# vigorbird/ORB_SLAM2_comment

Measured on AMD Instinct MI355X. Metric: frames/sec ORB extract+match, KITTI 1241×376 @1000 feat; HBM GB/s vs peak, higher is better.
Workload: dtype u8; 1 GPU; configs[1]+[2]+[3]: a global batch of 512 synthetic 1241x376 u8 frames per step, 512 per GPU, resident in HBM as (last, cur) pairs; per step ORB extract (nFeatures=1000, 8-level pyramid) of every frame + device-resident SearchByProjection(CurrentFrame, LastFrame, th=15, mono; projection prologue included) for every pair; monocular handles: mvImagePyramid[0] on demand (orbhip_extractor_set_lazy_lev; handles_per_gpu=3, stage_gates=0, global_batch=512, nfeatures=1000, levels=8, parallelism=pair-sharded x1

## Files before the change

orb_slam2_comment_amd/csrc/orbhip_extractor.hip:

```cpp
#include "orbhip_internal.h"
#include "rbrief_pattern.h"

#include <cfloat>
#include <climits>
#include <cmath>
#include <ctime>
#include <mutex>
#include <new>
#include <vector>

namespace orbhip {

static thread_local char g_err[512] = "";
void set_error(const char *fmt, ...)
{
    va_list ap;
    va_start(ap, fmt);
    vsnprintf(g_err, sizeof(g_err), fmt, ap);
    va_end(ap);
}

__device__ __forceinline__ int wave_reduce_add(int v) { return wave_sum(v); }

template <int T>
// ... 1081 lines not shown
                int spos = incl - surv_cnt;
                for (int i = i_lo; i < i_hi; ++i) {
                    const int r = S.rnk[i];
                    const bool split = r != 0xffff && r <= J;
                    if (!split) {
                        const int ni = Gc + spos++;
                        S.nmap[i] = ni;
                        S.x0[nxt][ni] = S.x0[cur][i]; S.x1[nxt][ni] = S.x1[cur][i];
                        S.y0[nxt][ni] = S.y0[cur][i]; S.y1[nxt][ni] = S.y1[cur][i];
                        S.cnt[nxt][ni] = S.cnt[cur][i];
                    } else {
                        S.nmap[i] = 0x40000000;
                        const int px0 = S.x0[cur][i], px1 = S.x1[cur][i], py0 = S.y0[cur][i], py1 = S.y1[cur][i];
                        const int mx = px0 + ((px1 - px0 + 1) >> 1), my = py0 + ((py1 - py0 + 1) >> 1);
                        int g = r > 0 ? S.cincl[r - 1] : 0;
#pragma unroll
                        for (int q = 0; q < 4; ++q) {
                            const int c = CC[4 * i + q];
                            if (c > 0) {
                                const int ni = Gc - 1 - g;
                                S.x0[nxt][ni] = (short)((q & 1) ? mx : px0);
                                S.x1[nxt][ni] = (short)((q & 1) ? px1 : mx);
                                S.y0[nxt][ni] = (short)((q & 2) ? my : py0);
                                S.y1[nxt][ni] = (short)((q & 2) ? py1 : my);
                                S.cnt[nxt][ni] = c;
                                CC[4 * i + q] = ni;
                                nToExpand += (c > 1);
                                ++g;
                            }
                        }
                    }
                }
            }
            nToExpand = wave_sum(nToExpand);
            const int n_new = Gc + (n - (m > 0 ? J + 1 : 0));
            int fin = 0, ph = phase;
            if (n_new >= N || n_new == prevSize) fin = 1;
            else if (phase == 1 && n_new + nToExpand * 3 > N) ph = 2;
            if (lane == 0) { S.vars[0] = n_new; S.vars[1] = fin; S.vars[2] = ph; }
            int *CN = S.ccnt[cb ^ 1];
            for (int i = lane; i < n_new * 4; i += 64) CN[i] = 0;
        }
        __syncthreads();
        OCT_STAMP(6);
        ++npass;
        if constexpr (REG) {
            oct_sweep<MAXN, T, false>(S, rkey, rlab, K, tid, cur, nxt, CC, S.ccnt[cb ^ 1], false, S.vars[1] == 0);
        } else {
            for (int k0 = 0; k0 < K; k0 += T * kOctU) {
                int nd[kOctU], mp[kOctU];
                uint32_t kv[kOctU];
#pragma unroll
                for (int u = 0; u < kOctU; ++u) {
                    const int k = k0 + u * T + tid;
                    nd[u] = k < K ? (int)knode(k) : 0;
                    kv[u] = k < K ? keys(k) : 0u;
                }
#pragma unroll
                for (int u = 0; u < kOctU; ++u) mp[u] = S.nmap[nd[u]];
                int bx0[kOctU], bx1[kOctU], by0[kOctU], by1[kOctU];
#pragma unroll
                for (int u = 0; u < kOctU; ++u) {
                    bx0[u] = S.x0[cur][nd[u]]; bx1[u] = S.x1[cur][nd[u]];
                    by0[u] = S.y0[cur][nd[u]]; by1[u] = S.y1[cur][nd[u]];
                }
#pragma unroll
                for (int u = 0; u < kOctU; ++u) {
                    const int k = k0 + u * T + tid;
                    if (k >= K) continue;
                    if (mp[u] & 0x40000000) {
                        const int x = kv[u] & 0xfff, y = (kv[u] >> 12) & 0xfff;
                        const int mx = bx0[u] + ((bx1[u] - bx0[u] + 1) >> 1), my = by0[u] + ((by1[u] - by0[u] + 1) >> 1);
                        knode(k) = (unsigned short)CC[4 * nd[u] + (x < mx ? 0 : 1) + (y < my ? 0 : 2)];
                    } else {
                        knode(k) = (unsigned short)mp[u];
                    }
                }
            }
        }
        OCT_STAMP(7);
        n = S.vars[0];
        finish = S.vars[1] != 0;
        phase = S.vars[2];
        cur = nxt;
        cb ^= 1;
    }
    __syncthreads();

    unsigned int *best = reinterpret_cast<unsigned int *>(S.ccnt[0]);
    for (int i = tid; i < n; i += T) best[i] = 0;
    __syncthreads();
    uint32_t *out = sel_kp + (size_t)b * G.kp_cap_total + L.kp_base;
    const int nout = min(n, L.kp_cap);
    if constexpr (REG) {
#pragma unroll
        for (int g = 0; g < kOctR / kOctU; ++g) {
            if (g * kOctU * T < K) {
#pragma unroll
                for (int u = 0; u < kOctU; ++u) {
                    const int k = (g * kOctU + u) * T + tid;
                    if (k < K) atomicMax(&best[oct_nd(rlab, g * kOctU + u)], ((rkey[g * kOctU + u] >> 24) << 24) | (0xffffffu - (uint32_t)k));
                }
            }
        }
        __syncthreads();
#pragma unroll
        for (int g = 0; g < kOctR / kOctU; ++g) {
            if (g * kOctU * T < K) {
                unsigned int bv[kOctU];
#pragma unroll
                for (int u = 0; u < kOctU; ++u) bv[u] = best[oct_nd(rlab, g * kOctU + u)];
#pragma unroll
                for (int u = 0; u < kOctU; ++u) {
                    const int k = (g * kOctU + u) * T + tid, nd = oct_nd(rlab, g * kOctU + u);
                    if (k < K && nd < nout && bv[u] == (((rkey[g * kOctU + u] >> 24) << 24) | (0xffffffu - (uint32_t)k)))
                        out[nd] = rkey[g * kOctU + u];
                }
            }
        }
    } else {
        for (int k0 = 0; k0 < K; k0 += T * kOctU) {
            int nd[kOctU];
            uint32_t kv[kOctU];
#pragma unroll
            for (int u = 0; u < kOctU; ++u) {
                const int k = k0 + u * T + tid;
                nd[u] = k < K ? (int)knode(k) : 0;
                kv[u] = k < K ? keys(k) : 0u;
            }
#pragma unroll
            for (int u = 0; u < kOctU; ++u) {
                const int k = k0 + u * T + tid;
                if (k < K) atomicMax(&best[nd[u]], ((kv[u] >> 24) << 24) | (0xffffffu - (uint32_t)k));
            }
        }
        __syncthreads();
        for (int i = tid; i < nout; i += T) out[i] = keys(0xffffffu - (best[i] & 0xffffffu));
    }
    if (tid == 0) {
        sel_cnt[b * ORBHIP_MAX_LEVELS + level] = nout;
        if (n > L.kp_cap) atomicExch(&frame_status[b], ORBHIP_E_CAPACITY);
    }
    OCT_STAMP(8);
#ifdef ORBHIP_DEVTOOLS
    if constexpr (STAMPS) {
        if (tid == 0 && level == 0) {
#pragma unroll
            for (int i = 0; i < 9; ++i) atomicAdd(&g_oct_stamps[i], tacc[i]);
            atomicAdd(&g_oct_stamps[9], (unsigned long long)npass);
            atomicAdd(&g_oct_stamps[10], 1ull);
            atomicAdd(&g_oct_stamps[11], (unsigned long long)K);
        }
    }
#endif
#undef OCT_STAMP
#undef keys
#undef knode
}

template <int MAXN, int T, bool STAMPS = false>
__global__ __launch_bounds__(T) __attribute__((amdgpu_waves_per_eu(MAXN == 512 && T == 512 ? 8 : 1))) void k_octree(PyrGeom G, const int *__restrict__ cell_cnt,
                                                const uint32_t *__restrict__ cell_kp,
                                                uint32_t *__restrict__ keys_ws,
                                                unsigned short *__restrict__ node_ws,
                                                uint32_t *__restrict__ sel_kp,
                                                int *__restrict__ sel_cnt, int *__restrict__ frame_status,
                                                const int reg_cap)
{
    __shared__ OctShared<MAXN> S;
    unsigned long long t0 = 0;
    if constexpr (STAMPS) t0 = stamp_now();
    int level, b;
    xcd_remap(level, b);
    const int tid = threadIdx.x;
    const LevelGeom L = G.lv[level];
    uint32_t *gkeys = keys_ws + (size_t)b * G.cand_cap_total + L.cand_base;
    unsigned short *gnode = node_ws + (size_t)b * G.cand_cap_total + L.cand_base;
    const int *ccnt_in = cell_cnt + (size_t)b * G.ncells_total + L.cell_base;
    const uint32_t *ckp_in = cell_kp + ((size_t)b * G.ncells_total + L.cell_base) * G.slot_cap;
    int tot;
    int K = 0;
    for (int c0 = 0; c0 < L.ncells; c0 += T) {
        int c = c0 + tid;
        int n = c < L.ncells ? ccnt_in[c] : 0;
        int base = block_excl_scan<T>(n, S.scan, &tot);
        if (c < L.ncells) S.ccnt[0][c] = K + base;
        K += tot;
    }
    K = __builtin_amdgcn_readfirstlane(K);
    if (K <= reg_cap)
        octree_body<MAXN, T, true, STAMPS>(S, G, L, level, b, K, ccnt_in, ckp_in, gkeys, gnode, sel_kp, sel_cnt, frame_status, t0);
    else
        octree_body<MAXN, T, false, STAMPS>(S, G, L, level, b, K, ccnt_in, ckp_in, gkeys, gnode, sel_kp, sel_cnt, frame_status, t0);
}

constexpr int kBIn = kBlurTH + 6;
constexpr int kBInW = 18;

__device__ __forceinline__ uint32_t mad24u(uint32_t a, uint32_t b, uint32_t c)
{
    uint32_t r;
    asm("v_mad_u32_u24 %0, %1, %2, %3" : "=v"(r) : "v"(a), "v"(b), "v"(c));
    return r;
}
__device__ __forceinline__ uint32_t sat_pk_u8(uint32_t v)
{
    uint32_t r;
    asm("v_sat_pk_u8_i16 %0, %1" : "=v"(r) : "v"(v));
    return r;
}

__global__ __launch_bounds__(256) void k_blur(const uint8_t *__restrict__ pyr, uint8_t *__restrict__ blur,
                                              PyrGeom G, const TileDesc *__restrict__ tiles, BlurW W)
{
    __shared__ uint32_t sin[kBIn * kBInW];
    __shared__ uint4 srow[(kBIn / 2) * (kBlurTW / 4)];
    int tile, fr;
    xcd_remap(tile, fr);
    const TileDesc t = tiles[tile];
    const LevelGeom L = G.lv[t.level];
    const size_t fo = (size_t)fr * G.frame_bytes + L.plane_off + (size_t)kEdge * L.pitch + kPadL;
    const uint8_t *roi = pyr + fo;
    uint8_t *out = blur + fo;
    const int x0 = t.tx * kBlurTW, y0 = t.ty * kBlurTH;
    const int rows = min(kBlurTH, L.h - y0);
    const int nin = rows + 6, npair = (nin + 1) >> 1;
    const int tid = threadIdx.x;
    const int gxmax = (L.w + 12) & ~3;
    {
        constexpr int U = (kBIn * kBInW + 255) / 256;
        uint32_t v[U];
#pragma unroll
        for (int u = 0; u < U; ++u) {
            const int i = min(u * 256 + tid, nin * kBInW - 1);
            const int r = (i * 3641) >> 16, c = i - r * kBInW;
            const int gy = min(y0 - 3 + r, L.h + kEdge - 1), gx = min(x0 - 4 + 4 * c, gxmax);
            v[u] = *reinterpret_cast<const uint32_t *>(roi + (ptrdiff_t)(__mul24(gy, L.pitch) + gx));
        }
#pragma unroll
        for (int u = 0; u < U; ++u) {
            const int i = u * 256 + tid;
            if (i < nin * kBInW) sin[i] = v[u];
        }
    }
    const uint32_t B0 = W.w[0], B1 = W.w[1], B2 = W.w[2], B3 = W.w[3], B4 = W.w[4], B5 = W.w[5], B6 = W.w[6];
    const uint32_t k0a = (B0 << 8) | (B1 << 16) | (B2 << 24), k0b = B3 | (B4 << 8) | (B5 << 16) | (B6 << 24);
    const uint32_t k1a = (B0 << 16) | (B1 << 24), k1b = B2 | (B3 << 8) | (B4 << 16) | (B5 << 24), k1c = B6;
    const uint32_t k2a = B0 << 24, k2b = B1 | (B2 << 8) | (B3 << 16) | (B4 << 24), k2c = B5 | (B6 << 8);
    const uint32_t k3b = B0 | (B1 << 8) | (B2 << 16) | (B3 << 24), k3c = B4 | (B5 << 8) | (B6 << 16);
    __syncthreads();
    for (int it = tid; it < npair * 16; it += 256) {
        const int pr = it >> 4, g = it & 15;
        uint32_t s[2][4];
#pragma unroll
        for (int h = 0; h < 2; ++h) {
            const uint32_t *p = &sin[madi24(min(2 * pr + h, nin - 1), kBInW, g)];
            const uint32_t d0 = p[0], d1 = p[1], d2 = p[2];
            s[h][0] = __builtin_amdgcn_udot4(d0, k0a, __builtin_amdgcn_udot4(d1, k0b, 0, false), false);
            s[h][1] = __builtin_amdgcn_udot4(d0, k1a, __builtin_amdgcn_udot4(d1, k1b, __builtin_amdgcn_udot4(d2, k1c, 0, false), false), false);
            s[h][2] = __builtin_amdgcn_udot4(d0, k2a, __builtin_amdgcn_udot4(d1, k2b, __builtin_amdgcn_udot4(d2, k2c, 0, false), false), false);
            s[h][3] = __builtin_amdgcn_udot4(d1, k3b, __builtin_amdgcn_udot4(d2, k3c, 0, false), false);
        }
        srow[it] = make_uint4(__builtin_amdgcn_perm(s[1][0], s[0][0], 0x05040100u), __builtin_amdgcn_perm(s[1][1], s[0][1], 0x05040100u),
                              __builtin_amdgcn_perm(s[1][2], s[0][2], 0x05040100u), __builtin_amdgcn_perm(s[1][3], s[0][3], 0x05040100u));
    }
    __syncthreads();
    const uint32_t w01 = (uint32_t)W.w[0] | ((uint32_t)W.w[1] << 16), w23 = (uint32_t)W.w[2] | ((uint32_t)W.w[3] << 16),
                   w45 = (uint32_t)W.w[4] | ((uint32_t)W.w[5] << 16), w12 = (uint32_t)W.w[1] | ((uint32_t)W.w[2] << 16),
                   w34 = (uint32_t)W.w[3] | ((uint32_t)W.w[4] << 16), w56 = (uint32_t)W.w[5] | ((uint32_t)W.w[6] << 16),
                   w6l = (uint32_t)W.w[6], w0h = (uint32_t)W.w[0] << 16;
    const int nprow = (rows + 1) >> 1;
    for (int it = tid; it < nprow * 16; it += 256) {
        const int p = it >> 4, g = it & 15;
        if (x0 + 4 * g >= L.w) continue;
        const uint4 P0 = srow[p * 16 + g], P1 = srow[(p + 1) * 16 + g], P2 = srow[(p + 2) * 16 + g], P3 = srow[(p + 3) * 16 + g];
        const uint32_t a0[4] = {P0.x, P0.y, P0.z, P0.w}, a1[4] = {P1.x, P1.y, P1.z, P1.w},
                       a2[4] = {P2.x, P2.y, P2.z, P2.w}, a3[4] = {P3.x, P3.y, P3.z, P3.w};
        uint32_t acce[4], acco[4];
#pragma unroll
        for (int j = 0; j < 4; ++j) {
            acce[j] = udot2(a0[j], w01, udot2(a1[j], w23, udot2(a2[j], w45, udot2(a3[j], w6l, 32768u))));
            acco[j] = udot2(a1[j], w12, udot2(a2[j], w34, udot2(a3[j], w56, udot2(a0[j], w0h, 32768u))));
        }
        const uint32_t rese = sat_pk_u8(__builtin_amdgcn_perm(acce[1], acce[0], 0x07060302u)) |
                              (sat_pk_u8(__builtin_amdgcn_perm(acce[3], acce[2], 0x07060302u)) << 16);
        const uint32_t reso = sat_pk_u8(__builtin_amdgcn_perm(acco[1], acco[0], 0x07060302u)) |
                              (sat_pk_u8(__builtin_amdgcn_perm(acco[3], acco[2], 0x07060302u)) << 16);
        uint8_t *o = out + (uint32_t)(__mul24(y0 + 2 * p, L.pitch) + x0 + 4 * g);
        *reinterpret_cast<uint32_t *>(o) = rese;
        if (2 * p + 1 < rows) *reinterpret_cast<uint32_t *>(o + L.pitch) = reso;
    }
}

constexpr int kWinRows = 43, kWinDw = 11;
constexpr int kWinRpi = 5;
constexpr int kWinLoads = 9;
constexpr int kWinWords = kWinRows * kWinDw + 7;
constexpr int kHPairs = 22, kHGroups = 10;

#ifndef ORBHIP_DESC_WAVES
#define ORBHIP_DESC_WAVES 7
#endif
constexpr int kDescWaveSlotsPerCu = 4 * ORBHIP_DESC_WAVES, kDescMinRounds = 6;
static int desc_per_wave(int kp_cap_total, int batch, int num_cus)
{
    const double slots = (double)num_cus * kDescWaveSlotsPerCu;
    for (int p = 4; p > 2; --p)
        if ((double)kp_cap_total * batch / p >= kDescMinRounds * slots) return p;
    return 2;
}

__global__ __launch_bounds__(256) __attribute__((amdgpu_waves_per_eu(ORBHIP_DESC_WAVES, ORBHIP_DESC_WAVES))) void k_describe_fused(const uint8_t *__restrict__ pyr, PyrGeom G,
                                                        const uint32_t *__restrict__ sel_kp,
                                                        const int *__restrict__ sel_cnt,
                                                        const int *__restrict__ desc_tab,
                                                        const float4 *__restrict__ patternf,
                                                        orbhip_keypoint *__restrict__ out_kp,
                                                        uint8_t *__restrict__ out_desc, int cap,
                                                        int *__restrict__ out_n, int *__restrict__ status, int per_wave, BlurW W,
                                                        const uint32_t *__restrict__ hitem_tab,
                                                        const uint8_t *__restrict__ images, int img_stride, size_t img_frame_stride)
{
    __shared__ uint32_t swin[4][kWinWords];
    __shared__ uint4 shsum[4][kHPairs * kHGroups];
    const int lane = threadIdx.x & 63;
    const int wv = __builtin_amdgcn_readfirstlane(threadIdx.x >> 6);
    int bx, b;
    xcd_remap(bx, b);
    int cw[4], uw[4], vw[4];
#pragma unroll
    for (int k = 0; k < 4; ++k) { cw[k] = desc_tab[k * 64 + lane]; uw[k] = desc_tab[256 + k * 64 + lane]; vw[k] = desc_tab[512 + k * 64 + lane]; }
    float4 pat[4];
#pragma unroll
    for (int j = 0; j < 4; ++j) pat[j] = patternf[j * 64 + lane];
    const int *cnts = sel_cnt + b * ORBHIP_MAX_LEVELS;
    int total = 0;
    for (int l = 0; l < G.nlevels; ++l) total += cnts[l];
    if (bx == 0 && wv == 0 && lane == 0) {
        out_n[b] = min(total, cap);
        if (total > cap && status) atomicExch(&status[b], ORBHIP_E_CAPACITY);
    }
    const uint32_t B0 = W.w[0], B1 = W.w[1], B2 = W.w[2], B3 = W.w[3], B4 = W.w[4], B5 = W.w[5], B6 = W.w[6];
    const uint32_t h0a = B0 | (B1 << 8) | (B2 << 16) | (B3 << 24), h0b = B4 | (B5 << 8) | (B6 << 16);
    const uint32_t h1a = (B0 << 8) | (B1 << 16) | (B2 << 24), h1b = B3 | (B4 << 8) | (B5 << 16) | (B6 << 24);
    const uint32_t h2a = (B0 << 16) | (B1 << 24), h2b = B2 | (B3 << 8) | (B4 << 16) | (B5 << 24), h2c = B6;
    const uint32_t h3a = B0 << 24, h3b = B1 | (B2 << 8) | (B3 << 16) | (B4 << 24), h3c = B5 | (B6 << 8);
    const uint32_t w01 = B0 | (B1 << 16), w23 = B2 | (B3 << 16), w45 = B4 | (B5 << 16), w12 = B1 | (B2 << 16),
                   w34 = B3 | (B4 << 16), w56 = B5 | (B6 << 16), w6l = B6, w0h = B0 << 16;
    const int srow = (lane * 373) >> 12, scol = lane - srow * kWinDw;
    const uint32_t hitems = hitem_tab[lane];
    uint32_t *win = swin[wv];
    uint4 *hs = shsum[wv];
  int level = 0, before = 0, mine = 0, kp_base = 0, kp_end = -1, pitch = 0;
  for (int kk = 0; kk < per_wave; ++kk) {
    const int slot = (bx * 4 + wv) * per_wave + kk;
    if (slot >= G.kp_cap_total) break;
    if (slot >= kp_end) {
        level = 0;
        for (int l = 1; l < G.nlevels; ++l) if (slot >= G.lv[l].kp_base) level = l;
        before = 0; mine = 0;
        for (int l = 0; l < G.nlevels; ++l) {
            const int c = cnts[l];
            if (l < level) before += c;
            if (l == level) mine = c;
        }
        kp_base = G.lv[level].kp_base; kp_end = kp_base + G.lv[level].kp_cap; pitch = G.lv[level].pitch;
    }
    const int i = slot - kp_base;
    if (i >= mine) continue;
    const int oidx = before + i;
    if (oidx >= cap) continue;

    const uint32_t kv = sel_kp[(size_t)b * G.kp_cap_total + slot];
    const int kx = (int)(kv & 0xfff) + 16, ky = (int)((kv >> 12) & 0xfff) + 16;
    const int resp = (int)(kv >> 24);
    uint32_t wvv[kWinLoads];
    const bool from_img = images != nullptr && level == 0;
    const bool inside = kx >= 21 && kx + 22 < G.lv[0].w && ky >= 21 && ky + 21 < G.lv[0].h;
    if (from_img && !inside) {
        const uint8_t *ib = images + (size_t)b * img_frame_stride;
        uint32_t cx[4];
#pragma unroll
        for (int k = 0; k < 4; ++k) cx[k] = (uint32_t)reflect101(kx - 21 + 4 * scol + k, G.lv[0].w);
#pragma unroll
        for (int u = 0; u < kWinLoads; ++u) {
            wvv[u] = 0u;
            if (lane < kWinRpi * kWinDw && (u < kWinLoads - 1 || srow < kWinRows - (kWinLoads - 1) * kWinRpi)) {
                const uint8_t *rp = ib + (size_t)((uint32_t)reflect101(ky - 21 + srow + u * kWinRpi, G.lv[0].h) * (uint32_t)img_stride);
                wvv[u] = (uint32_t)rp[cx[0]] | ((uint32_t)rp[cx[1]] << 8) | ((uint32_t)rp[cx[2]] << 16) | ((uint32_t)rp[cx[3]] << 24);
            }
        }
    } else {
        const int wpitch = from_img ? img_stride : pitch;
        const uint8_t *wb = from_img
            ? images + (size_t)b * img_frame_stride + (size_t)(ky - 21) * img_stride + (kx - 21)
            : pyr + (size_t)b * G.frame_bytes + G.lv[level].plane_off + (size_t)kEdge * pitch + kPadL + (size_t)(ky - 21) * pitch + (kx - 21);
        const uint32_t voff = (uint32_t)(__mul24(srow, wpitch) + 4 * scol);
#pragma unroll
        for (int u = 0; u < kWinLoads; ++u) {
            wvv[u] = 0u;
            if (lane < kWinRpi * kWinDw && (u < kWinLoads - 1 || srow < kWinRows - (kWinLoads - 1) * kWinRpi))
                __builtin_memcpy(&wvv[u], wb + (uint32_t)(u * kWinRpi * wpitch) + voff, 4);
        }
    }
    __builtin_amdgcn_wave_barrier();
    if (lane < kWinRpi * kWinDw) {
        uint32_t *dd = win + (srow * kWinDw + scol);
#pragma unroll
        for (int u = 0; u < kWinLoads; ++u)
            if (u < kWinLoads - 1 || srow < kWinRows - (kWinLoads - 1) * kWinRpi) dd[u * kWinRpi * kWinDw] = wvv[u];
    }
    __builtin_amdgcn_wave_barrier();
    int m10 = 0, m01 = 0;
#pragma unroll
    for (int k = 0; k < 4; ++k) {
        const int d = (int)(win[cw[k]] ^ 0x80808080u);
        m10 = __builtin_amdgcn_sdot4(d, uw[k], m10, false);
        m01 = __builtin_amdgcn_sdot4(d, vw[k], m01, false);
    }
#pragma unroll 1
    for (int q = 0; q < 3; ++q) {
        const int it = (int)((hitems >> (8 * q)) & 0xffu);
        const int pr = (it * 205) >> 11, g = it - pr * kHGroups;
        uint32_t s[2][4];
#pragma unroll
        for (int h = 0; h < 2; ++h) {
            const uint32_t *p = &win[madi24(min(2 * pr + h, kWinRows - 1), kWinDw, g)];
            const uint32_t d0 = p[0], d1 = p[1], d2 = p[2];
            s[h][0] = __builtin_amdgcn_udot4(d0, h0a, __builtin_amdgcn_udot4(d1, h0b, 0, false), false);
            s[h][1] = __builtin_amdgcn_udot4(d0, h1a, __builtin_amdgcn_udot4(d1, h1b, 0, false), false);
            s[h][2] = __builtin_amdgcn_udot4(d0, h2a, __builtin_amdgcn_udot4(d1, h2b, __builtin_amdgcn_udot4(d2, h2c, 0, false), false), false);
            s[h][3] = __builtin_amdgcn_udot4(d0, h3a, __builtin_amdgcn_udot4(d1, h3b, __builtin_amdgcn_udot4(d2, h3c, 0, false), false), false);
        }
        hs[it] = make_uint4(__builtin_amdgcn_perm(s[1][0], s[0][0], 0x05040100u), __builtin_amdgcn_perm(s[1][1], s[0][1], 0x05040100u),
                            __builtin_amdgcn_perm(s[1][2], s[0][2], 0x05040100u), __builtin_amdgcn_perm(s[1][3], s[0][3], 0x05040100u));
    }
    m10 = wave_reduce_add(m10);
    m01 = wave_reduce_add(m01);
    const float angle = fast_atan2_deg((float)m01, (float)m10);
    const float factorPI = (float)(3.14159265358979323846 / 180.f);
    float a, bsn;
    det_sincos(__fmul_rn(angle, factorPI), &a, &bsn);
    __builtin_amdgcn_wave_barrier();
    const uint32_t *hd = reinterpret_cast<const uint32_t *>(hs);
    auto round18 = [](float t) -> int {
        return (int)(__float_as_uint(__fadd_rn(t, 12582912.0f)) - (0x4B400000u - 18u));
    };
    uint32_t vw0, vw1, vw2, vw3, vx0, vx1, vx2, vx3;
    asm("v_mov_b32 %0, %1" : "=v"(vw0) : "s"(w01)); asm("v_mov_b32 %0, %1" : "=v"(vx0) : "s"(w01 ^ w0h));
    asm("v_mov_b32 %0, %1" : "=v"(vw1) : "s"(w23)); asm("v_mov_b32 %0, %1" : "=v"(vx1) : "s"(w23 ^ w12));
    asm("v_mov_b32 %0, %1" : "=v"(vw2) : "s"(w45)); asm("v_mov_b32 %0, %1" : "=v"(vx2) : "s"(w45 ^ w34));
    asm("v_mov_b32 %0, %1" : "=v"(vw3) : "s"(w6l)); asm("v_mov_b32 %0, %1" : "=v"(vx3) : "s"(w6l ^ w56));
    auto blurred = [&](int R, int C) -> int {
        const uint32_t *p = hd + madi24(R >> 1, kHGroups * 4, C);
        const uint32_t d0 = p[0], d1 = p[kHGroups * 4], d2 = p[2 * kHGroups * 4], d3 = p[3 * kHGroups * 4];
        const uint32_t om = 0u - (uint32_t)(R & 1);
        const uint32_t acc = udot2(d0, vw0 ^ (om & vx0), udot2(d1, vw1 ^ (om & vx1), udot2(d2, vw2 ^ (om & vx2),
                                   udot2(d3, vw3 ^ (om & vx3), 32768u))));
        return min((int)(acc >> 16), 255);
    };
    unsigned long long bits[4];
    int t0v[4], t1v[4];
#pragma unroll
    for (int j = 0; j < 4; ++j) {
        const float px0 = pat[j].x, py0 = pat[j].y, px1 = pat[j].z, py1 = pat[j].w;
        const int r0 = round18(__fadd_rn(__fmul_rn(px0, bsn), __fmul_rn(py0, a)));
        const int c0 = round18(__fsub_rn(__fmul_rn(px0, a), __fmul_rn(py0, bsn)));
        const int r1 = round18(__fadd_rn(__fmul_rn(px1, bsn), __fmul_rn(py1, a)));
        const int c1 = round18(__fsub_rn(__fmul_rn(px1, a), __fmul_rn(py1, bsn)));
        t0v[j] = blurred(r0, c0);
        t1v[j] = blurred(r1, c1);
    }
#pragma unroll
    for (int j = 0; j < 4; ++j) bits[j] = __ballot(t0v[j] < t1v[j]);
    if (lane < 4) {
        unsigned long long v = lane == 0 ? bits[0] : lane == 1 ? bits[1] : lane == 2 ? bits[2] : bits[3];
        reinterpret_cast<unsigned long long *>(out_desc + ((size_t)b * cap + oidx) * 32)[lane] = v;
    }
    if (lane == 0) {
        orbhip_keypoint kp;
        float fx = (float)kx, fy = (float)ky;
        const float scale = G.lv[level].scale;
        if (level != 0) { fx = __fmul_rn(fx, scale); fy = __fmul_rn(fy, scale); }
        kp.x = fx; kp.y = fy; kp.size = (float)G.lv[level].patch; kp.angle = angle; kp.response = (float)resp;
        kp.octave = level; kp.class_id = -1;
        out_kp[(size_t)b * cap + oidx] = kp;
    }
  }
}

__global__ void k_zero_status(int *status, int n)
{
    int i = blockIdx.x * blockDim.x + threadIdx.x;
    if (i < n) status[i] = 0;
}

}

using namespace orbhip;

#ifdef ORBHIP_DEVTOOLS
#define ORBHIP_STAGE_MASK(e) ((e)->stage_mask)
#else
#define ORBHIP_STAGE_MASK(e) 31
#endif

static int cv_round(double v) { return (int)lrint(v); }

static void drop_graph(orbhip_extractor *e)
{
    if (e->graph_exec) (void)hipGraphExecDestroy(e->graph_exec);
    e->graph_exec = nullptr; e->graph_batch = 0; e->graph_cap = 0;
}
static void free_geometry(orbhip_extractor *e)
{
    drop_graph(e);
    (void)hipFree(e->d_cells); (void)hipFree(e->d_cells2); (void)hipFree(e->d_tiles); (void)hipFree(e->d_pyrtab);
    e->d_cells = nullptr; e->d_cells2 = nullptr; e->d_tiles = nullptr; e->d_pyrtab = nullptr;
    e->bound = false;
}
static void free_batch(orbhip_extractor *e)
{
    drop_graph(e);
    (void)hipFree(e->d_pyr); (void)hipFree(e->d_blur); (void)hipFree(e->d_cell_cnt); (void)hipFree(e->d_cell_kp);
    (void)hipFree(e->d_keys); (void)hipFree(e->d_knode); (void)hipFree(e->d_sel); (void)hipFree(e->d_sel_cnt); (void)hipFree(e->d_status);
    e->d_pyr = e->d_blur = nullptr; e->d_cell_cnt = nullptr; e->d_cell_kp = nullptr; e->d_keys = nullptr;
    e->d_knode = nullptr; e->d_sel = nullptr; e->d_sel_cnt = nullptr; e->d_status = nullptr;
    (void)hipFree(e->d_gray); e->d_gray = nullptr; e->gray_cap = 0;
    e->batch_cap = 0;
    e->blur_valid = false;
}

static void host_resize_coef(int d, double scale, int slen, bool clamp_both, int &s0, int &s1, int &c0, int &c1)
{
#pragma clang fp contract(off)
    const double fd = ((double)d + 0.5) * scale;
    float f = (float)(fd - 0.5);
    int s = (int)floorf(f);
    f = f - (float)s;
    if (clamp_both) {
        s0 = s < 0 ? 0 : (s < slen ? s : slen - 1);
        s1 = s + 1 < 0 ? 0 : (s + 1 < slen ? s + 1 : slen - 1);
    } else {
        if (s < 0) { f = 0.f; s = 0; }
        if (s >= slen - 1) { f = 0.f; s = slen - 1; }
        s0 = s; s1 = s + 1;
    }
    const float g = 1.f - f;
    c0 = (int)lrintf(g * 2048.f);
    c1 = (int)lrintf(f * 2048.f);
}
static int host_reflect101(int p, int len)
{
    if (p < 0) p = -p;
    if (p >= len) p = 2 * (len - 1) - p;
    return p;
}
static void pyr_chunks(PyrLevelTab &T, int rows_per_unit)
{
    T.nchunks = (T.words + 63) / 64;
    T.chunk_w = (T.words + T.nchunks - 1) / T.nchunks;
    T.rcp_chunks = T.nchunks > 1 ? (uint32_t)(((1ull << 32) + (unsigned)T.nchunks - 1) / (unsigned)T.nchunks) : 0u;
    T.units = ((T.prows + rows_per_unit - 1) / rows_per_unit) * T.nchunks;
}

static int build_pyr_tables(orbhip_extractor *e)
{
    const PyrGeom &G = e->G;
    std::vector<uint8_t> blob;
    auto put = [&blob](const void *p, size_t n) {
        const size_t at = (blob.size() + 63) & ~(size_t)63;
        blob.resize(at + n);
        memcpy(blob.data() + at, p, n);
        return at;
    };
    size_t off_row[ORBHIP_MAX_LEVELS] = {0}, off_col[ORBHIP_MAX_LEVELS] = {0}, off_lo[ORBHIP_MAX_LEVELS] = {0};
    for (int l = 0; l < G.nlevels; ++l) {
        const LevelGeom &L = G.lv[l];
        PyrLevelTab &T = e->ptab[l];
        memset(&T, 0, sizeof(T));
        T.prows = L.prows; T.pitch = L.pitch; T.plane_off = L.plane_off;
        e->ptab_rows[l] = false;
        if (l == 0) {
            T.words = L.pitch >> 4;
            T.src_h = L.h;
            std::vector<PyrCopyCol> col(T.words);
            std::vector<uint32_t> lo(T.words);
            for (int g = 0; g < T.words; ++g) {
                int rk[16], base = 1 << 30;
                for (int k = 0; k < 16; ++k) {
                    const int x = g * 16 - kPadL + k;
                    rk[k] = (x >= -kEdge && x < L.w + kEdge) ? host_reflect101(x, L.w) : -1;
                    if (rk[k] >= 0) base = std::min(base, rk[k]);
                }
                if (base == (1 << 30)) base = 0;
                base = std::min(base, L.w - 16);
                lo[g] = (uint32_t)base;
                for (int j = 0; j < 4; ++j) {
                    uint32_t a = 0, b = 0;
                    for (int k = 0; k < 4; ++k) {
                        const int idx = rk[4 * j + k] < 0 ? -1 : rk[4 * j + k] - base;
                        a |= (uint32_t)((idx >= 0 && idx < 8) ? idx : 0x0c) << (8 * k);
                        b |= (uint32_t)((idx >= 8 && idx < 16) ? idx - 8 : 0x0c) << (8 * k);
                    }
                    col[g].selA[j] = a; col[g].selB[j] = b;
                }
            }
            pyr_chunks(T, kPyrRows);
            off_col[l] = put(col.data(), col.size() * sizeof(PyrCopyCol));
            off_lo[l] = put(lo.data(), lo.size() * sizeof(uint32_t));
            e->ptab_rows[l] = true;
            continue;
        }
        const LevelGeom &P = G.lv[l - 1];
        const double sx = 1. / ((double)L.w / P.w), sy = 1. / ((double)L.h / P.h);
        T.words = (kPadL + L.w + kEdge + 3) >> 2;
        T.src_h = P.h; T.src_pitch = P.pitch;
        T.src_off = P.plane_off + (unsigned)(kEdge * P.pitch + kPadL);
        std::vector<PyrCol> col(T.words);
        std::vector<uint32_t> lo(T.words);
        bool ok = P.w >= 8;
        for (int pw = 0; pw < T.words && ok; ++pw) {
            int sxk[4], a0[4], a1[4], lo_ = 1 << 30, hi_ = -1;
            bool valid[4];
            for (int k = 0; k < 4; ++k) {
                const int x = pw * 4 - kPadL + k;
                valid[k] = x >= -kEdge && x < L.w + kEdge;
                sxk[k] = 0; a0[k] = a1[k] = 0;
                if (!valid[k]) continue;
                int s1;
                host_resize_coef(host_reflect101(x, L.w), sx, P.w, false, sxk[k], s1, a0[k], a1[k]);
                lo_ = std::min(lo_, sxk[k]); hi_ = std::max(hi_, sxk[k]);
            }
            if (hi_ < 0) { lo_ = 0; hi_ = 0; }
            if (hi_ - lo_ > 6) { ok = false; break; }
            lo_ = std::min(lo_, P.w - 8);
            lo[pw] = (uint32_t)lo_;
            for (int k = 0; k < 4; ++k) {
                if (!valid[k]) { col[pw].sel[k] = 0x0c0c0c0cu; col[pw].alv[k] = 0; continue; }
                const int rel = sxk[k] - lo_;
                int rel1 = rel + 1;
                if (sxk[k] + 1 > P.w - 1) { rel1 = rel; if (a1[k] != 0) ok = false; }
                if (rel < 0 || rel1 > 7) ok = false;
                col[pw].sel[k] = 0x0c000c00u | (uint32_t)rel | ((uint32_t)rel1 << 16);
                col[pw].alv[k] = (uint32_t)a0[k] | ((uint32_t)a1[k] << 16);
            }
        }
        if (!ok) continue;
        std::vector<PyrRow> row(L.prows);
        for (int py = 0; py < L.prows; ++py) {
            int s0, s1, b0, b1;
            host_resize_coef(host_reflect101(py - kEdge, L.h), sy, P.h, true, s0, s1, b0, b1);
            row[py].s0 = s0; row[py].s1 = s1; row[py].B0 = (uint32_t)b0 << 12; row[py].B1 = (uint32_t)b1 << 12;
        }
        pyr_chunks(T, kPyrRows);
        off_row[l] = put(row.data(), row.size() * sizeof(PyrRow));
        off_col[l] = put(col.data(), col.size() * sizeof(PyrCol));
        off_lo[l] = put(lo.data(), lo.size() * sizeof(uint32_t));
        e->ptab_rows[l] = true;
    }
    ORBHIP_HIP_CHECK(hipMalloc(&e->d_pyrtab, blob.size() + 64));
    ORBHIP_HIP_CHECK(hipMemcpyAsync(e->d_pyrtab, blob.data(), blob.size(), hipMemcpyHostToDevice, e->stream));
    ORBHIP_HIP_CHECK(hipStreamSynchronize(e->stream));
    for (int l = 0; l < G.nlevels; ++l) {
        if (!e->ptab_rows[l]) continue;
        PyrLevelTab &T = e->ptab[l];
        T.row = reinterpret_cast<const PyrRow *>(e->d_pyrtab + off_row[l]);
        T.col = e->d_pyrtab + off_col[l];
        T.lo = reinterpret_cast<const uint32_t *>(e->d_pyrtab + off_lo[l]);
    }
    return ORBHIP_OK;
}

static FastCell make_fast_cell(const PyrGeom &G, const CellDesc &c, int img_stride)
{
    const LevelGeom &Lc = G.lv[c.level];
    FastCell f; memset(&f, 0, sizeof(f));
    const int a = kFastLead, gxb = c.x0 - a, sw = c.x1 - c.x0, shh = c.y1 - c.y0;
    if (img_stride > 0 && c.level == 0) {
        f.src_off = (unsigned)(c.y0 * img_stride + gxb - 4);
        f.pitch = (unsigned short)img_stride; f.img = 1;
    } else {
        f.src_off = Lc.plane_off + (unsigned)((kEdge + c.y0) * Lc.pitch + kPadL + gxb - 4);
        f.pitch = (unsigned short)Lc.pitch;
    }
    f.sw = (unsigned char)sw; f.sh = (unsigned char)shh; f.a = (unsigned char)a;
    f.kpx = (short)(c.offx - 4 - a); f.kpy = (short)(c.offy + 3);
    const int dwc = sw - 6, c_lo = a + 7, c_hi = c_lo + dwc;
    const int ngrp = dwc > 0 ? ((c_hi - 1) >> 2) - (c_lo >> 2) + 1 : 1;
    f.magic = ((1u << 18) + ngrp - 1) / ngrp;
    return f;
}

static int bind_geometry(orbhip_extractor *e, int rows, int cols)
{
    if (e->bound && e->G.rows == rows && e->G.cols == cols) return ORBHIP_OK;
    ORBHIP_HIP_CHECK(hipSetDevice(e->device));
    ORBHIP_HIP_CHECK(hipStreamSynchronize(e->stream));
    free_geometry(e);
    free_batch(e);
    PyrGeom &G = e->G;
    memset(&G, 0, sizeof(G));
    G.nlevels = e->nlevels; G.rows = rows; G.cols = cols; G.ini_th = e->iniTh; G.min_th = e->minTh;
    e->cells.clear(); e->tiles.clear();
    unsigned off = 0;
    int kp_base = 0, cand_base = 0, slot_cap = 1;
    for (int l = 0; l < e->nlevels; ++l) {
        LevelGeom &L = G.lv[l];
        const float scale = e->isf[l];
        L.w = cv_round((float)cols * scale);
        L.h = cv_round((float)rows * scale);
        if (L.w < 2 * kEdge + 2 || L.h < 2 * kEdge + 2 || L.w > 4000 || L.h > 4000) {
            set_error("level %d is %dx%d: unsupported (need 40..4000 px per side)", l, L.w, L.h);
            return ORBHIP_E_SIZE;
        }
        L.pitch = (kPadL + L.w + kEdge + 63) & ~63;
        L.prows = L.h + 2 * kEdge;
        L.plane_off = off;
        off += (unsigned)L.pitch * L.prows;
        off = (off + 255u) & ~255u;
        L.maxBX = L.w - kEdge + 3; L.maxBY = L.h - kEdge + 3;
        L.quota = e->nfeat[l];
        L.patch = (int)(kPatchSize * e->sf[l]);
        L.scale = e->sf[l];
        const int minB = kEdge - 3;
        const float width = (float)(L.maxBX - minB), height = (float)(L.maxBY - minB);
        const float W = 30;
        const int nCols = (int)(width / W), nRows = (int)(height / W);
        L.cell_base = (int)e->cells.size();
        if (nCols >= 1 && nRows >= 1) {
            const int wCell = (int)ceilf(width / nCols), hCell = (int)ceilf(height / nRows);
            if (wCell + 6 > kSubMax || hCell + 6 > kSubMax) { set_error("cell too large"); return ORBHIP_E_SIZE; }
            for (int i = 0; i < nRows; ++i) {
                const float iniY = (float)(minB + i * hCell);
                float maxY = iniY + hCell + 6;
                if (iniY >= L.maxBY - 3) continue;
                if (maxY > L.maxBY) maxY = (float)L.maxBY;
                for (int j = 0; j < nCols; ++j) {
                    const float iniX = (float)(minB + j * wCell);
                    float maxX = iniX + wCell + 6;
                    if (iniX >= L.maxBX - 6) continue;
                    if (maxX > L.maxBX) maxX = (float)L.maxBX;
                    CellDesc c;
                    c.level = (short)l; c.x0 = (short)iniX; c.y0 = (short)iniY; c.x1 = (short)maxX; c.y1 = (short)maxY;
                    c.offx = (short)(j * wCell); c.offy = (short)(i * hCell); c.pad = 0;
                    e->cells.push_back(c);
                    int dw = c.x1 - c.x0 - 6, dh = c.y1 - c.y0 - 6;
                    if (dw > 0 && dh > 0) slot_cap = std::max(slot_cap, ((dw + 1) / 2) * ((dh + 1) / 2));
                }
            }
        }
        L.ncells = (int)e->cells.size() - L.cell_base;
        const int bw = L.maxBX - minB, bh = L.maxBY - minB;
        int nIni = bh > 0 ? (int)roundf((float)bw / bh) : 0;
        if (nIni < 1) nIni = 1;
        L.nIni = nIni;
        L.hX = (float)bw / nIni;
        L.kp_cap = std::max(L.quota + 3, 4 * nIni);
        L.kp_base = kp_base; kp_base += L.kp_cap;
        for (int ty = 0; ty * kBlurTH < L.h; ++ty)
            for (int tx = 0; tx * kBlurTW < L.w; ++tx) {
                TileDesc t; t.level = (short)l; t.tx = (short)tx; t.ty = (short)ty; t.pad = 0;
                e->tiles.push_back(t);
            }
    }
    {
        int msh = 7, mdh = 1, mdw = 1, mndw = 2;
        for (const CellDesc &c : e->cells) {
            msh = std::max(msh, c.y1 - c.y0);
            mdh = std::max(mdh, c.y1 - c.y0 - 6);
            mdw = std::max(mdw, c.x1 - c.x0 - 6);
            mndw = std::max(mndw, (kFastLead + (c.x1 - c.x0) + 3) >> 2);
        }
        FastLds &F2 = e->fast_lds;
        const int need = mndw + 1;
        F2.strideW = need <= 11 ? 11 : need <= 13 ? 13 : need <= 15 ? 15 : need <= 17 ? 17 : 21;
        if (need > 21) { set_error("cell geometry exceeds the FAST kernel limits"); return ORBHIP_E_SIZE; }
        F2.scoreW = F2.strideW - 2;
        F2.score_words = (mdh + 2) * F2.scoreW;
        {
            const int lpr = F2.strideW <= 16 ? 16 : 32, rpi = 64 / lpr, rows_batch = rpi * kFastStageU;
            const int rows = ((msh + rows_batch - 1) / rows_batch) * rows_batch;
            F2.img_words = rows * F2.strideW;
        }
        {
            const int full = mdw * mdh, row_px = 4 * ((mdw + 3) >> 2), fixed = (F2.img_words + F2.score_words) * 4;
            int cap = full;
            for (int wgs = 32; wgs >= 4; wgs -= 4) {
                const int share = kFastLdsPerCu / wgs / kFastLdsGranule * kFastLdsGranule;
                const int room = (share - fixed) / 2 - 2;
// ... 1138 lines not shown
```

Baseline: 296,000 frames/s.

## Batch orientation moments for a wave's keypoints ahead of descriptor loop

The describe kernel now gathers the orientation-moment pixels for all of a wave's keypoints (up to four) straight from global memory in one pass. It reduces the moments, then computes atan2 and sincos once, with each keypoint held in its own lane. The per-keypoint loop then pulls level, offset, angle and sin/cos through readlane, and only builds the shared window for the blur and BRIEF tests. This takes the serial moment-reduce and trig chain out of each keypoint's critical path and lets the global loads for several keypoints be in flight together. The cost is extra redundant global reads of the moment pixels and more live registers under a fixed waves-per-EU bound, which could cause spills.

```diff
diff --git a/orb_slam2_comment_amd/csrc/orbhip_extractor.hip b/orb_slam2_comment_amd/csrc/orbhip_extractor.hip
--- a/orb_slam2_comment_amd/csrc/orbhip_extractor.hip
+++ b/orb_slam2_comment_amd/csrc/orbhip_extractor.hip
@@ -1407,10 +1407,11 @@
 #define ORBHIP_DESC_WAVES 7
 #endif
 constexpr int kDescWaveSlotsPerCu = 4 * ORBHIP_DESC_WAVES, kDescMinRounds = 6;
+constexpr int kDescGroup = 4;
 static int desc_per_wave(int kp_cap_total, int batch, int num_cus)
 {
     const double slots = (double)num_cus * kDescWaveSlotsPerCu;
-    for (int p = 4; p > 2; --p)
+    for (int p = kDescGroup; p > 2; --p)
         if ((double)kp_cap_total * batch / p >= kDescMinRounds * slots) return p;
     return 2;
 }
@@ -1432,12 +1433,14 @@
     const int wv = __builtin_amdgcn_readfirstlane(threadIdx.x >> 6);
     int bx, b;
     xcd_remap(bx, b);
-    int cw[4], uw[4], vw[4];
-#pragma unroll
-    for (int k = 0; k < 4; ++k) { cw[k] = desc_tab[k * 64 + lane]; uw[k] = desc_tab[256 + k * 64 + lane]; vw[k] = desc_tab[512 + k * 64 + lane]; }
-    float4 pat[4];
-#pragma unroll
-    for (int j = 0; j < 4; ++j) pat[j] = patternf[j * 64 + lane];
+    int crow[4], ccol[4], uw[4], vw[4];
+#pragma unroll
+    for (int k = 0; k < 4; ++k) {
+        const int cwk = desc_tab[k * 64 + lane];
+        crow[k] = (cwk * 373) >> 12;
+        ccol[k] = 4 * (cwk - crow[k] * kWinDw);
+        uw[k] = desc_tab[256 + k * 64 + lane]; vw[k] = desc_tab[512 + k * 64 + lane];
+    }
     const int *cnts = sel_cnt + b * ORBHIP_MAX_LEVELS;
     int total = 0;
     for (int l = 0; l < G.nlevels; ++l) total += cnts[l];
@@ -1457,32 +1460,96 @@
     uint32_t *win = swin[wv];
     uint4 *hs = shsum[wv];
   int level = 0, before = 0, mine = 0, kp_base = 0, kp_end = -1, pitch = 0;
-  for (int kk = 0; kk < per_wave; ++kk) {
-    const int slot = (bx * 4 + wv) * per_wave + kk;
-    if (slot >= G.kp_cap_total) break;
-    if (slot >= kp_end) {
-        level = 0;
-        for (int l = 1; l < G.nlevels; ++l) if (slot >= G.lv[l].kp_base) level = l;
-        before = 0; mine = 0;
-        for (int l = 0; l < G.nlevels; ++l) {
-            const int c = cnts[l];
-            if (l < level) before += c;
-            if (l == level) mine = c;
-        }
-        kp_base = G.lv[level].kp_base; kp_end = kp_base + G.lv[level].kp_cap; pitch = G.lv[level].pitch;
-    }
-    const int i = slot - kp_base;
-    if (i >= mine) continue;
-    const int oidx = before + i;
-    if (oidx >= cap) continue;
-
-    const uint32_t kv = sel_kp[(size_t)b * G.kp_cap_total + slot];
+  {
+    constexpr int kk0 = 0;
+    int s_kv = 0, s_meta = -1, s_m10 = 0, s_m01 = 0, s_off = 0, s_pitch = 0;
+    uint32_t md[kDescGroup][4];
+#pragma unroll
+    for (int s = 0; s < kDescGroup; ++s) {
+#pragma unroll
+        for (int k = 0; k < 4; ++k) md[s][k] = 0x80808080u;
+        const int slot = (bx * 4 + wv) * per_wave + kk0 + s;
+        if (kk0 + s >= per_wave || slot >= G.kp_cap_total) continue;
+        if (slot >= kp_end) {
+            level = 0;
+            for (int l = 1; l < G.nlevels; ++l) if (slot >= G.lv[l].kp_base) level = l;
+            before = 0; mine = 0;
+            for (int l = 0; l < G.nlevels; ++l) {
+                const int c = cnts[l];
+                if (l < level) before += c;
+                if (l == level) mine = c;
+            }
+            kp_base = G.lv[level].kp_base; kp_end = kp_base + G.lv[level].kp_cap; pitch = G.lv[level].pitch;
+        }
+        const int i = slot - kp_base;
+        if (i >= mine) continue;
+        const int oidx = before + i;
+        if (oidx >= cap) continue;
+        const uint32_t kv = sel_kp[(size_t)b * G.kp_cap_total + slot];
+        const int kx = (int)(kv & 0xfff) + 16, ky = (int)((kv >> 12) & 0xfff) + 16;
+        const bool from_img = images != nullptr && level == 0;
+        const bool inside = kx >= 21 && kx + 22 < G.lv[0].w && ky >= 21 && ky + 21 < G.lv[0].h;
+        const int wpitch = from_img ? img_stride : pitch;
+        const uint32_t woff = from_img ? (uint32_t)((ky - 21) * img_stride + (kx - 21))
+                                       : G.lv[level].plane_off + (uint32_t)((kEdge + ky - 21) * pitch + kPadL + (kx - 21));
+        if (lane == s) {
+            s_kv = (int)kv; s_off = (int)woff; s_pitch = wpitch;
+            s_meta = level | (from_img ? 16 : 0) | (from_img && !inside ? 32 : 0) | (oidx << 6);
+        }
+        if (from_img && !inside) {
+            const uint8_t *ib = images + (size_t)b * img_frame_stride;
+#pragma unroll
+            for (int k = 0; k < 4; ++k) {
+                const uint8_t *rp = ib + (size_t)((uint32_t)reflect101(ky - 21 + crow[k], G.lv[0].h) * (uint32_t)img_stride);
+                uint32_t d = 0;
+#pragma unroll
+                for (int j = 0; j < 4; ++j) d |= (uint32_t)rp[reflect101(kx - 21 + ccol[k] + j, G.lv[0].w)] << (8 * j);
+                md[s][k] = d;
+            }
+        } else {
+            const uint8_t *wb = (from_img ? images + (size_t)b * img_frame_stride : pyr + (size_t)b * G.frame_bytes) + woff;
+#pragma unroll
+            for (int k = 0; k < 4; ++k) __builtin_memcpy(&md[s][k], wb + (uint32_t)(__mul24(crow[k], wpitch) + ccol[k]), 4);
+        }
+    }
+#pragma unroll
+    for (int s = 0; s < kDescGroup; ++s) {
+        if (kk0 + s >= per_wave) continue;
+        int m10 = 0, m01 = 0;
+#pragma unroll
+        for (int k = 0; k < 4; ++k) {
+            const int d = (int)(md[s][k] ^ 0x80808080u);
+            m10 = __builtin_amdgcn_sdot4(d, uw[k], m10, false);
+            m01 = __builtin_amdgcn_sdot4(d, vw[k], m01, false);
+        }
+        const int r10 = wave_reduce_add(m10), r01 = wave_reduce_add(m01);
+        if (lane == s) { s_m10 = r10; s_m01 = r01; }
+    }
+    const float s_angle = fast_atan2_deg((float)s_m01, (float)s_m10);
+    float s_a, s_b;
+    {
+        const float factorPI = (float)(3.14159265358979323846 / 180.f);
+        det_sincos(__fmul_rn(s_angle, factorPI), &s_a, &s_b);
+    }
+    float4 pat[4];
+#pragma unroll
+    for (int j = 0; j < 4; ++j) pat[j] = patternf[j * 64 + lane];
+  for (int kk = kk0; kk < min(kk0 + kDescGroup, per_wave); ++kk) {
+    const int meta = __builtin_amdgcn_readlane(s_meta, kk - kk0);
+    if (meta < 0) continue;
+    const int lvl = meta & 15, oidx = meta >> 6;
+    const uint32_t kv = (uint32_t)__builtin_amdgcn_readlane(s_kv, kk - kk0);
+    const float angle = __int_as_float(__builtin_amdgcn_readlane(__float_as_int(s_angle), kk - kk0));
+    float a, bsn;
+    asm("v_mov_b32 %0, %1" : "=v"(a) : "s"(__builtin_amdgcn_readlane(__float_as_int(s_a), kk - kk0)));
+    asm("v_mov_b32 %0, %1" : "=v"(bsn) : "s"(__builtin_amdgcn_readlane(__float_as_int(s_b), kk - kk0)));
+    const int wpitch = __builtin_amdgcn_readlane(s_pitch, kk - kk0);
+    const uint32_t woff = (uint32_t)__builtin_amdgcn_readlane(s_off, kk - kk0);
     const int kx = (int)(kv & 0xfff) + 16, ky = (int)((kv >> 12) & 0xfff) + 16;
     const int resp = (int)(kv >> 24);
     uint32_t wvv[kWinLoads];
-    const bool from_img = images != nullptr && level == 0;
-    const bool inside = kx >= 21 && kx + 22 < G.lv[0].w && ky >= 21 && ky + 21 < G.lv[0].h;
-    if (from_img && !inside) {
+    const bool from_img = (meta & 16) != 0;
+    if (meta & 32) {
         const uint8_t *ib = images + (size_t)b * img_frame_stride;
         uint32_t cx[4];
 #pragma unroll
@@ -1496,10 +1563,7 @@
             }
         }
     } else {
-        const int wpitch = from_img ? img_stride : pitch;
-        const uint8_t *wb = from_img
-            ? images + (size_t)b * img_frame_stride + (size_t)(ky - 21) * img_stride + (kx - 21)
-            : pyr + (size_t)b * G.frame_bytes + G.lv[level].plane_off + (size_t)kEdge * pitch + kPadL + (size_t)(ky - 21) * pitch + (kx - 21);
+        const uint8_t *wb = (from_img ? images + (size_t)b * img_frame_stride : pyr + (size_t)b * G.frame_bytes) + woff;
         const uint32_t voff = (uint32_t)(__mul24(srow, wpitch) + 4 * scol);
 #pragma unroll
         for (int u = 0; u < kWinLoads; ++u) {
@@ -1516,13 +1580,6 @@
             if (u < kWinLoads - 1 || srow < kWinRows - (kWinLoads - 1) * kWinRpi) dd[u * kWinRpi * kWinDw] = wvv[u];
     }
     __builtin_amdgcn_wave_barrier();
-    int m10 = 0, m01 = 0;
-#pragma unroll
-    for (int k = 0; k < 4; ++k) {
-        const int d = (int)(win[cw[k]] ^ 0x80808080u);
-        m10 = __builtin_amdgcn_sdot4(d, uw[k], m10, false);
-        m01 = __builtin_amdgcn_sdot4(d, vw[k], m01, false);
-    }
 #pragma unroll 1
     for (int q = 0; q < 3; ++q) {
         const int it = (int)((hitems >> (8 * q)) & 0xffu);
@@ -1540,12 +1597,6 @@
         hs[it] = make_uint4(__builtin_amdgcn_perm(s[1][0], s[0][0], 0x05040100u), __builtin_amdgcn_perm(s[1][1], s[0][1], 0x05040100u),
                             __builtin_amdgcn_perm(s[1][2], s[0][2], 0x05040100u), __builtin_amdgcn_perm(s[1][3], s[0][3], 0x05040100u));
     }
-    m10 = wave_reduce_add(m10);
-    m01 = wave_reduce_add(m01);
-    const float angle = fast_atan2_deg((float)m01, (float)m10);
-    const float factorPI = (float)(3.14159265358979323846 / 180.f);
-    float a, bsn;
-    det_sincos(__fmul_rn(angle, factorPI), &a, &bsn);
     __builtin_amdgcn_wave_barrier();
     const uint32_t *hd = reinterpret_cast<const uint32_t *>(hs);
     auto round18 = [](float t) -> int {
@@ -1585,12 +1636,13 @@
     if (lane == 0) {
         orbhip_keypoint kp;
         float fx = (float)kx, fy = (float)ky;
-        const float scale = G.lv[level].scale;
-        if (level != 0) { fx = __fmul_rn(fx, scale); fy = __fmul_rn(fy, scale); }
-        kp.x = fx; kp.y = fy; kp.size = (float)G.lv[level].patch; kp.angle = angle; kp.response = (float)resp;
-        kp.octave = level; kp.class_id = -1;
+        const float scale = G.lv[lvl].scale;
+        if (lvl != 0) { fx = __fmul_rn(fx, scale); fy = __fmul_rn(fy, scale); }
+        kp.x = fx; kp.y = fy; kp.size = (float)G.lv[lvl].patch; kp.angle = angle; kp.response = (float)resp;
+        kp.octave = lvl; kp.class_id = -1;
         out_kp[(size_t)b * cap + oidx] = kp;
     }
+  }
   }
 }
 
```

New measurement: 281,200 frames/s. 5.0% lower.
